# arihantb2/direct_lidar_odometry

Measured on AMD Instinct MI355X. Metric: gicp_iterations_per_sec, higher is better.
Workload: dtype f64

## Files before the change

direct_lidar_odometry_amd/csrc/ngicp_pass_group.inc:

```
#ifndef NG_ROBUST
#define NG_ROBUST false
#define NG_ROBUST_DEFAULTED
#endif
  for (int item = group * 4 + wave; item < a.n_batches; item = a.n_batches) {
    typedef const int __attribute__((address_space(4))) * ConstBatchPtr;
    ConstBatchPtr brec = (ConstBatchPtr)(unsigned long long)a.batches + 2 * (size_t)item;
    const int2 it = make_int2(brec[0], brec[1]);
    typedef const float __attribute__((address_space(4))) * ConstBoxPtr;
    const unsigned int far_word = (unsigned int)((ConstBatchPtr)(unsigned long long)a.batch_far)[item >> 2];
    const bool far_before = ((far_word >> (8 * (item & 3))) & 0xffu) != 0;
    ConstBoxPtr bbp = (ConstBoxPtr)(unsigned long long)a.batch_boxes + 6 * (size_t)item;
    const float bb_c0 = bbp[0], bb_c1 = bbp[1], bb_c2 = bbp[2], bb_h0 = bbp[3], bb_h1 = bbp[4], bb_h2 = bbp[5];
    const int qbase = it.x, qcount = it.y, batch = item;
    float mybest = 3.4028234664e38f;
    int mypos = -1;
    const int i = qbase + lane;
    const bool mine = lane < qcount;
    NG_STAMP(1);
    const bool have_prev = NG_HAVE_LIN != 0;
    float4 sp = make_float4(0.f, 0.f, 0.f, 0.f);
    int j_old = -1;
    float4 bp_old = make_float4(0.f, 0.f, 0.f, 0.f);
    double k4 = 0.0;
    double Mold[6] = {0, 0, 0, 0, 0, 0};
    if (mine) {
      sp = a.qpts[i];
      if (have_prev) {
        bp_old = tpt_old[i];
        j_old = __float_as_int(bp_old.w);
      }
      if (do_err) {
        const double* M = mahal_old + (size_t)i * 6;
#pragma unroll
        for (int e = 0; e < 6; ++e) Mold[e] = M[e];
      }
    }
    int Y0 = 0, Z0 = 0, wy = 1, grow = 0, nlive = 0;
    int b0x = 0, b0y = 0, b0z = 0, b1x = 0, b1y = 0, b1z = 0;
    bool list_rows = false;
    int rs[kStageRowsPerLane], rn[kStageRowsPerLane], rho[kStageRowsPerLane], ryz[kStageRowsPerLane], rk[kStageRowsPerLane];
    if (do_lin && !(a.mode & 8) && a.stage_grow >= 2 && (have_prev ? far_before : (a.mode & 32) != 0)) {
      {
        const float bcx = bb_c0, bcy = bb_c1, bcz = bb_c2, bhx = bb_h0, bhy = bb_h1, bhz = bb_h2;
        const float3 m = transform_point_rowmajor_f(Tf, bcx, bcy, bcz);
        const float mx = m.x, my = m.y, mz = m.z;
        const float pad = 1e-3f * g.h;
        const float ex = (fabsf(Tf[0]) * bhx + fabsf(Tf[1]) * bhy) + fabsf(Tf[2]) * bhz + pad + 4e-6f * (fabsf(mx) + bhx + bhy + bhz);
        const float ey = (fabsf(Tf[4]) * bhx + fabsf(Tf[5]) * bhy) + fabsf(Tf[6]) * bhz + pad + 4e-6f * (fabsf(my) + bhx + bhy + bhz);
        const float ez = (fabsf(Tf[8]) * bhx + fabsf(Tf[9]) * bhy) + fabsf(Tf[10]) * bhz + pad + 4e-6f * (fabsf(mz) + bhx + bhy + bhz);
        cell_coords(g, mx - ex, my - ey, mz - ez, b0x, b0y, b0z);
        cell_coords(g, mx + ex, my + ey, mz + ez, b1x, b1y, b1z);
      }
      int rows, X0 = 0, XS = 1;
      for (grow = a.stage_grow;; --grow) {
        X0 = max(b0x - grow, 0);
        Y0 = max(b0y - grow, 0);
        Z0 = max(b0z - grow, 0);
        const int X1 = min(b1x + grow, g.nx - 1), Y1 = min(b1y + grow, g.ny - 1), Z1 = min(b1z + grow, g.nz - 1);
        XS = X1 - X0 + 1;
        wy = Y1 - Y0 + 1;
        rows = wy * (Z1 - Z0 + 1);
        if ((rows <= kStageRows && XS <= kStageXs) || grow == 2) break;
      }
      if (rows <= kStageRows && XS <= kStageXs) {
        int sv[kStageRowsPerLane], ev[kStageRowsPerLane], ka[kStageRowsPerLane], kb[kStageRowsPerLane];
#pragma unroll
        for (int k = 0; k < kStageRowsPerLane; ++k) {
          const int r = lane + 64 * k;
          const bool has = r < rows;
          const int ry = Y0 + (has ? r : 0) % wy, rz = Z0 + (has ? r : 0) / wy;
          const int* rowp = a.tgt_cell_start + ((rz * g.ny + ry) * g.nx + X0);
          sv[k] = rowp[0];
          ev[k] = rowp[XS];
          ka[k] = rowp[b0x - X0];
          kb[k] = rowp[b1x + 1 - X0];
          rho[k] = max(max(b0y - ry, ry - b1y), max(max(b0z - rz, rz - b1z), 0));
          ryz[k] = ry | (rz << 16);
        }
        static_assert(kStageRowsPerLane == 4, "the four rows of a lane, spelled out for the compiler");
        asm volatile("" ::"v"(sv[0]), "v"(sv[1]), "v"(sv[2]), "v"(sv[3]), "v"(kb[0]), "v"(kb[1]), "v"(kb[2]), "v"(kb[3]));
#pragma unroll
        for (int k = 0; k < kStageRowsPerLane; ++k) {
          const bool has = lane + 64 * k < rows;
          rs[k] = sv[k];
          rn[k] = has ? ev[k] - sv[k] : 0;
          rk[k] = min(ka[k] - sv[k], 0xffff) | (min(kb[k] - sv[k], 0xffff) << 16);
        }
        list_rows = true;
      }
    }
    if (mine) {
      if (do_err && j_old >= 0) {
        const double ax = (double)sp.x, ay = (double)sp.y, az = (double)sp.z;
        const double tax = R[0] * ax + R[1] * ay + R[2] * az + t[0];
        const double tay = R[3] * ax + R[4] * ay + R[5] * az + t[1];
        const double taz = R[6] * ax + R[7] * ay + R[8] * az + t[2];
        const double ex = (double)bp_old.x - tax, ey = (double)bp_old.y - tay, ez = (double)bp_old.z - taz;
        if constexpr (NG_ROBUST) {
          k4 = err_term_robust(a.robust_kind, a.robust_c, a.robust_c2, ex, ey, ez, Mold);
        } else {
        const double m00 = Mold[0], m01 = Mold[1], m02 = Mold[2], m11 = Mold[3], m12 = Mold[4], m22 = Mold[5];
        const double mex = m00 * ex + m01 * ey + m02 * ez;
        const double mey = m01 * ex + m11 * ey + m12 * ez;
        const double mez = m02 * ex + m12 * ey + m22 * ez;
        k4 = ex * mex + ey * mey + ez * mez;
        }
      }
    }

    if (do_lin && (a.mode & 8)) {
      mypos = (qbase + lane) % 1000;
      mybest = 0.01f;
    } else if (do_lin) {
      const int qi = qbase + grp;
      const bool qok = grp < qcount;
      const float qpx = __shfl(sp.x, grp), qpy = __shfl(sp.y, grp), qpz = __shfl(sp.z, grp);
      const int jp = __shfl(j_old, grp);
      float4 bpo;
      bpo.x = __shfl(bp_old.x, grp); bpo.y = __shfl(bp_old.y, grp); bpo.z = __shfl(bp_old.z, grp); bpo.w = 0.f;
      float qx = 0.f, qy = 0.f, qz = 0.f;
      int cx = 0, cy = 0, cz = 0;
      if (qok) {
        const float3 q = transform_point_rowmajor_f(Tf, qpx, qpy, qpz);
        qx = q.x, qy = q.y, qz = q.z;
        cell_coords(g, qx, qy, qz, cx, cy, cz);
      }
      float best = 3.4028234664e38f;
      int pos = -1;
      if (qok && jp >= 0) {
        best = sqdist(qx, qy, qz, bpo);
        pos = jp;
      }
      NG_STAMP(2);
      bool listed = false;
      if (list_rows) {
        {
          wave_lds_sync();
          for (int lev = 0; lev <= grow; ++lev) {
#pragma unroll
            for (int k = 0; k < kStageRowsPerLane; ++k) {
              const bool on = rn[k] > 0 && rho[k] == lev;
              const unsigned long long m = __ballot(on);
              if (on) S.live[nlive + __popcll(m & ((1ull << lane) - 1ull))] = make_int4(ryz[k], rn[k], rs[k], rk[k]);
              nlive += __popcll(m);
            }
          }
          listed = true;
        }
      }
      NG_STAMP(3);
      if (a.dbg_stamps && lane == 0) {
        unsigned long long* d = a.dbg_stamps + (size_t)(blockIdx.x * 4 + wave) * kStampStride;
        d[10] = (unsigned long long)(listed ? grow : 0);
        d[11] = (unsigned long long)nlive;
        d[12] = (unsigned long long)qcount;
        d[13] = (unsigned long long)((b1x - b0x + 1) | ((b1y - b0y + 1) << 8) | ((b1z - b0z + 1) << 16));
      }
      bool went_far = false;
      const bool in_box = qok && listed && cx >= b0x && cx <= b1x && cy >= b0y && cy <= b1y && cz >= b0z && cz <= b1z;
      unsigned int dbg_g1 = 0, dbg_g2 = 0;
      auto pack_key = [](float d, int p) { return ((unsigned long long)__float_as_uint(d) << 32) | (unsigned int)p; };
      if (qok && sub == 0) {
        if (in_box) ++nstaged;
        S.qtab[grp] = make_float4(qx, qy, qz, 0.f);
        S.qkey[grp] = pack_key(best, pos);
      }
      if (lane == 0) S.q_tail = 0, S.q_head = 0;
      if (a.dbg_qstats && lane < 32) S.qstat[lane][0] = S.qstat[lane][1] = S.qstat[lane][2] = 0;
      wave_lds_sync();
      if (qok) {
        const float lim = fminf(best, a.gate_sq_f);
        constexpr int kRowsPerLane = (9 + G - 1) / G;
        struct alignas(4) Bounds4 { int v[4]; };
        Bounds4 bnd[kRowsPerLane], bxs[kRowsPerLane];
        float gap[kRowsPerLane];
        int code[kRowsPerLane];
#pragma unroll
        for (int k = 0; k < kRowsPerLane; ++k) {
          const int order = sub + k * G;
          const int tt = order == 0 ? 4 : (order < 5 ? 2 * order - 1 : (order == 5 ? 0 : (order == 6 ? 2 : (order == 7 ? 6 : 8))));
          const int z = cz + tt / 3 - 1, y = cy + tt % 3 - 1;
          code[k] = -1;
          gap[k] = 0.f;
          bnd[k] = Bounds4{{0, 0, 0, 0}};
          bxs[k] = Bounds4{{0, 0, 0, 0}};
          if (order < 9 && z >= 0 && z < g.nz && y >= 0 && y < g.ny) {
            gap[k] = row_gap_sq(g, y, z, cy, cz, qy, qz);
            if (gap[k] <= lim) {
              code[k] = tt;
              bnd[k] = *reinterpret_cast<const Bounds4*>(a.tgt_cell_start + ((z * g.ny + y) * g.nx + cx - 1));
              if (a.tgt_cell_box) bxs[k] = *reinterpret_cast<const Bounds4*>(a.tgt_cell_box + ((z * g.ny + y) * g.nx + cx - 1));
            }
          }
        }
        const float fx = fminf(fmaxf((qx - (g.ox + (float)cx * g.h)) * g.inv_h, 0.f), 1.f);
        int ntail = 0;
#pragma unroll
        for (int k = 0; k < kRowsPerLane; ++k) {
          const int s0 = cx > 0 ? bnd[k].v[0] : bnd[k].v[1], e0 = cx < g.nx - 1 ? bnd[k].v[3] : bnd[k].v[2];
          bool has = code[k] >= 0 && e0 > s0;
          if (has && a.tgt_cell_box) {
            unsigned int ub = (unsigned int)bxs[k].v[1];
            if (cx > 0) ub = cell_box_union(ub, (unsigned int)bxs[k].v[0]);
            if (cx < g.nx - 1) ub = cell_box_union(ub, (unsigned int)bxs[k].v[2]);
            gap[k] = fmaxf(gap[k], box_gap_sq(g, cy + code[k] % 3 - 1, cz + code[k] / 3 - 1, ub, qy, qz));
            has = gap[k] <= lim;
          }
          const unsigned long long hm = __ballot(has);
          if (has) {
            const int m = (jp >= s0 && jp < e0) ? jp : bnd[k].v[1] + (int)(fx * (float)(bnd[k].v[2] - bnd[k].v[1]));
            const int slot = ntail + __popcll(hm & ((1ull << lane) - 1ull));
            S.unit_q[slot] = grp | (code[k] << 5) | (min(max(m - s0, 0), (1 << 22) - 1) << 9);
            S.unit_s[slot] = s0;
            S.unit_e[slot] = e0;
            S.unit_g[slot] = gap[k];
          }
          ntail += __popcll(hm);
        }
        if (lane == 0) S.q_tail = ntail, S.q_head = 64 / kWalkLanes;
      }
      wave_lds_sync();
      int li_pre = sub;
      bool pre_far = false;
#if NGICP_PRE_FAR
      if (listed) {
        if (in_box) {
          const float b1 = unexplored_bound_sq(g, qx, qy, qz, cx, cy, cz, 1);
          pre_far = !(best <= b1 || b1 >= a.gate_sq_f);
        }
        if (__any(pre_far)) {
          if (pre_far) {
            const float lim = fminf(best, a.gate_sq_f);
            const float fxb = fminf(fmaxf((qx - (g.ox + (float)b0x * g.h)) / ((float)(b1x + 1 - b0x) * g.h), 0.f), 1.f);
            for (; li_pre < nlive; li_pre += G) {
              const int4 rec = S.live[li_pre];
              const float gp = row_gap_sq(g, rec.x & 0xffff, rec.x >> 16, cy, cz, qy, qz);
              if (gp > lim) continue;
              const int slot = atomicAdd(&S.q_tail, 1);
              if (slot >= kUnitCap) break;
              const int k0 = rec.w & 0xffff, k1 = (int)((unsigned int)rec.w >> 16);
              S.unit_q[slot] = grp | (9 << 5) | (min(max(k0 + (int)(fxb * (float)(k1 - k0)), 0), (1 << 22) - 1) << 9);
              S.unit_s[slot] = rec.z;
              S.unit_e[slot] = rec.z + rec.y;
              S.unit_g[slot] = gp;
            }
          }
          wave_lds_sync();
        }
      }
#endif
      NG_STAMP(16);
      {
        const int tail = min(S.q_tail, kUnitCap);
        unsigned int popped = 0;
        constexpr int kWalkers = 64 / kWalkLanes;
        const int ql = lane % kWalkLanes;
        auto next_unit = [&]() {
          if (tail <= kWalkers) return tail;
          if constexpr (kWalkLanes == 1) {
            return atomicAdd(&S.q_head, 1);
          } else {
            int nu = 0;
            if (ql == 0) nu = atomicAdd(&S.q_head, 1);
            return quad_perm_i<0x00>(nu);
          }
        };
        for (int u = lane / kWalkLanes; u < tail; u = next_unit()) {
          ++popped;
          const int uq = S.unit_q[u], qs = uq & 31, s0 = S.unit_s[u], e0 = S.unit_e[u];
          const float gyz = S.unit_g[u];
          const float4 q = S.qtab[qs];
          const unsigned long long k0 = S.qkey[qs];
          float ub = __uint_as_float((unsigned int)(k0 >> 32));
          int up = (int)(unsigned int)k0;
          if (gyz > fminf(ub, a.gate_sq_f)) continue;
          const unsigned int c_before = ncand;
          const unsigned int steps_before1 = dbg_g1;
          if constexpr (kWalkLanes == 1) scan_global_outward<kWin, kSideStep>(a.tgt3, s0, e0, s0 + (uq >> 9), q.x, q.y, q.z, gyz, a.gate_sq_f, ub, up, ncand, dbg_g1);
          else scan_quad_outward<kWin, kSideStep>(a.tgt3, s0, e0, s0 + (uq >> 9), q.x, q.y, q.z, gyz, a.gate_sq_f, ub, up, ncand, dbg_g1, ql);
          if (ql == 0) {
            if (a.dbg_qstats) atomicAdd(reinterpret_cast<int*>(a.dbg_qstats + a.n_src) + min((int)((dbg_g1 - steps_before1) & 0xffff), 63), 1);
            atomicMin(&S.qkey[qs], pack_key(ub, up));
            if (a.dbg_qstats) {
              atomicAdd(&S.qstat[qs][0], (int)(ncand - c_before));
              atomicAdd(&S.qstat[qs][1], 1);
            }
          }
        }
        NG_STAMP(17);
        if (a.dbg_stamps) {
          unsigned long long* d = a.dbg_stamps + (size_t)(blockIdx.x * 4 + wave) * kStampStride;
          atomicMax(&d[18], (unsigned long long)popped);
          if (lane == 0) d[19] = (unsigned long long)tail;
        }
      }
      wave_lds_sync();
      if (qok) {
        const unsigned long long k1 = S.qkey[grp];
        best = __uint_as_float((unsigned int)(k1 >> 32));
        pos = (int)(unsigned int)k1;
      }
      NG_STAMP(4);
      float bound1 = 0.f;
      if (qok) {
        bound1 = unexplored_bound_sq(g, qx, qy, qz, cx, cy, cz, 1);
        went_far = !(best <= bound1 || bound1 >= a.gate_sq_f);
      }
      const unsigned int dbg_c1 = ncand;
      unsigned int dbg_rows = 0;
      const bool need_far = in_box && went_far;
      if (listed && __any(need_far && (!pre_far || li_pre < nlive))) {
        int li = pre_far ? li_pre : sub;
        bool more = need_far;
        for (;;) {
          if (lane == 0) S.q_tail = 0, S.q_head = 0;
          wave_lds_sync();
          if (more) {
            const float lim = fminf(best, a.gate_sq_f);
            for (; li < nlive; li += G) {
              const int4 rec = S.live[li];
              if (row_gap_sq(g, rec.x & 0xffff, rec.x >> 16, cy, cz, qy, qz) > lim) continue;
              const int slot = atomicAdd(&S.q_tail, 1);
              if (slot >= kUnitCap) break;
              S.unit_q[slot] = grp | (li << 5);
              ++dbg_rows;
            }
            more = li < nlive;
          }
          wave_lds_sync();
          {
            const int tail = min(S.q_tail, kUnitCap);
            const int ql = lane % kWalkLanes;
            for (;;) {
              int u = 0;
              if (ql == 0) u = atomicAdd(&S.q_head, 1);
              if constexpr (kWalkLanes > 1) u = quad_perm_i<0x00>(u);
              if (u >= tail) break;
              const int unit = S.unit_q[u], qs = unit & 31;
              const int4 rec = S.live[unit >> 5];
              const float4 q = S.qtab[qs];
              int ux, uy, uz;
              cell_coords(g, q.x, q.y, q.z, ux, uy, uz);
              const float gyz = row_gap_sq(g, rec.x & 0xffff, rec.x >> 16, uy, uz, q.y, q.z);
              const unsigned long long k0 = S.qkey[qs];
              float ub = __uint_as_float((unsigned int)(k0 >> 32));
              int up = (int)(unsigned int)k0;
              if (gyz > fminf(ub, a.gate_sq_f)) continue;
              const int s0 = rec.z + (rec.w & 0xffff), e0 = rec.z + (int)((unsigned int)rec.w >> 16);
              const float frac3 = fminf(fmaxf((q.x - (g.ox + (float)b0x * g.h)) / ((float)(b1x + 1 - b0x) * g.h), 0.f), 1.f);
              const unsigned int c_before = ncand;
              const unsigned int steps_before2 = dbg_g2;
              if constexpr (kWalkLanes == 1) scan_global_outward<kWin, kSideStep>(a.tgt3, rec.z, rec.z + rec.y, s0 + (int)(frac3 * (float)(e0 - s0)), q.x, q.y, q.z, gyz, a.gate_sq_f, ub, up, ncand, dbg_g2);
              else scan_quad_outward<kWin, kSideStep>(a.tgt3, rec.z, rec.z + rec.y, s0 + (int)(frac3 * (float)(e0 - s0)), q.x, q.y, q.z, gyz, a.gate_sq_f, ub, up, ncand, dbg_g2, ql);
              if (ql == 0) {
                if (a.dbg_qstats) atomicAdd(reinterpret_cast<int*>(a.dbg_qstats + a.n_src) + 64 + min((int)((dbg_g2 - steps_before2) & 0xffff), 63), 1);
                atomicMin(&S.qkey[qs], pack_key(ub, up));
                if (a.dbg_qstats) {
                  atomicAdd(&S.qstat[qs][2], (int)(ncand - c_before));
                  atomicAdd(&S.qstat[qs][1], 1 << 16);
                }
              }
            }
          }
          wave_lds_sync();
          if (in_box) {
            const unsigned long long k1 = S.qkey[grp];
            best = __uint_as_float((unsigned int)(k1 >> 32));
            pos = (int)(unsigned int)k1;
          }
          if (!__any(more)) break;
        }
      }
      NG_STAMP(5);
      if (a.dbg_stamps && qok) {
        unsigned long long* d = a.dbg_stamps + (size_t)(blockIdx.x * 4 + wave) * kStampStride;
        atomicMax(&d[14], ((unsigned long long)(dbg_g2 & 0xffff) << 48) | ((unsigned long long)(dbg_g2 >> 16) << 32) | ((unsigned long long)dbg_rows << 16) | (ncand - dbg_c1));
        atomicMax(&d[15], ((unsigned long long)(dbg_g1 & 0xffff) << 48) | ((unsigned long long)(dbg_g1 >> 16) << 32) | dbg_c1);
      }
      const unsigned int c_before_shells = ncand;
      if (qok) nn_shells<G>(g, a.tgt3, a.tgt_cell_start, qx, qy, qz, cx, cy, cz, a.gate_sq_f, sub, need_far ? grow : 1, best, pos, ncand);
      if (a.dbg_qstats) {
        if (qok) atomicAdd(&S.qstat[grp][2], (int)(ncand - c_before_shells));
        wave_lds_sync();
        if (qok && sub == 0) a.dbg_qstats[qi] = make_int4(S.qstat[grp][0], S.qstat[grp][1], S.qstat[grp][2], (went_far ? 1 : 0) | (in_box ? 2 : 0) | (pos >= 0 ? 4 : 0));
      }
      {
        const bool any_far = __any(went_far);
        if (lane == 0) a.batch_far[batch] = any_far ? 1 : 0;
      }
      NG_STAMP(6);
      const int src_lane = (lane % B) * G;
      mybest = __shfl(best, src_lane);
      mypos = __shfl(pos, src_lane);
    }
    double acc[kNumSums];
#pragma unroll
    for (int v = 0; v < kNumSums; ++v) acc[v] = 0.0;
    if ((a.mode & 16) && mine) {
      tpt_new[i] = make_float4(0.f, 0.f, 0.f, __int_as_float(mypos));
      acc[27] += (double)mybest;
    } else if (mine) {
      const double ax = (double)sp.x, ay = (double)sp.y, az = (double)sp.z;
      const double tax = R[0] * ax + R[1] * ay + R[2] * az + t[0];
      const double tay = R[3] * ax + R[4] * ay + R[5] * az + t[1];
      const double taz = R[6] * ax + R[7] * ay + R[8] * az + t[2];

      acc[28] += k4;
      if (do_lin) {
        const int pos = mypos;
        const bool valid = (pos >= 0) && ((double)mybest < a.gate_sq);
        if (!valid) tpt_new[i] = make_float4(0.f, 0.f, 0.f, __int_as_float(-1));
        if (valid) {
          ++nvalid;
          const double* CB = a.cov_tgt + (size_t)pos * 6;
          const double* CA = a.cov_src + (size_t)__float_as_int(sp.w) * 6;
          const Xyz bp = a.tgt3[pos];
          double ca[6];
#pragma unroll
          for (int e = 0; e < 6; ++e) ca[e] = CA[e];
          tpt_new[i] = make_float4(bp.x, bp.y, bp.z, __int_as_float(pos));
          double rcr[6], M[6];
          rotate_sym(R, ca, rcr);
#pragma unroll
          for (int e = 0; e < 6; ++e) rcr[e] = CB[e] + rcr[e];
          inv3_sym(rcr, M);
          double* Mo = mahal_new + (size_t)i * 6;
#pragma unroll
          for (int e = 0; e < 6; ++e) Mo[e] = M[e];

          const double ex = (double)bp.x - tax, ey = (double)bp.y - tay, ez = (double)bp.z - taz;
          if constexpr (NG_ROBUST) lin_terms_robust(acc, a.robust_kind, a.robust_c, a.robust_c2, tax, tay, taz, ex, ey, ez, M);
          else lin_terms(acc, tax, tay, taz, ex, ey, ez, M);
        }
      }
    }
    {
      double* red = S.red;
      double out = 0.0;
#pragma unroll
      for (int half = 0; half < 2; ++half) {
        wave_lds_sync();
        if ((lane >> 4) == half) {
#pragma unroll
          for (int v = 0; v < kNumSums; ++v) red[(lane & 15) * 30 + v] = acc[v];
        }
        wave_lds_sync();
        if (lane < kNumSums)
          for (int l = 0; l < 16; ++l) out += red[l * 30 + lane];
      }
      if (lane < kNumSums) wave_total += out;
    }
  }

  NG_STAMP(7);
  {
    wave_lds_sync();
    unsigned int* cnt = reinterpret_cast<unsigned int*>(S.red);
    cnt[lane] = ncand;
    cnt[64 + lane] = nvalid;
    cnt[128 + lane] = nstaged;
    wave_lds_sync();
    if (lane >= kNumSums && lane < kNumSlots) {
      unsigned int sum = 0;
      for (int l = 0; l < 64; ++l) sum += cnt[(lane - kNumSums) * 64 + l];
      wave_total = (double)sum;
    }
    if (lane < kNumSlots) lds[wave][lane] = wave_total;
  }
  NG_STAMP(8);
  __syncthreads();
  NG_STAMP(9);
  if (threadIdx.x < kNumSlots) {
    const int v = threadIdx.x;
    const double val = ((lds[0][v] + lds[1][v]) + lds[2][v]) + lds[3][v];
    if (FUSED) __hip_atomic_store(a.partials + (size_t)group * kNumSlots + v, val, __ATOMIC_RELAXED, __HIP_MEMORY_SCOPE_AGENT);
    else a.partials[(size_t)group * kNumSlots + v] = val;
  }
  if (a.dbg_span && threadIdx.x == 0) {
    unsigned long long* d = a.dbg_span + (size_t)blockIdx.x * 4;
    d[1] = __builtin_amdgcn_s_memrealtime();
    d[2] = (unsigned long long)__builtin_amdgcn_s_getreg((31 << 11) | 4) | ((unsigned long long)__builtin_amdgcn_s_getreg((31 << 11) | 20) << 32);
    d[3] = (unsigned long long)(unsigned int)group;
  }
  if (a.grp_cost && threadIdx.x == 0) {
    const int cost = (int)min((__builtin_amdgcn_s_memtime() - t_start) >> 4, 0x7fffffffull);
    if (FUSED) __hip_atomic_store(a.grp_cost + group, cost, __ATOMIC_RELAXED, __HIP_MEMORY_SCOPE_AGENT);
    else a.grp_cost[group] = cost;
  }
#ifdef NG_ROBUST_DEFAULTED
#undef NG_ROBUST
#undef NG_ROBUST_DEFAULTED
#endif
```

direct_lidar_odometry_amd/csrc/ngicp_search.h:

```cpp
#pragma once
#include "ngicp_grid.h"

namespace ngk {

struct alignas(4) Xyz { float x, y, z; };
__device__ __forceinline__ float sqdist(float qx, float qy, float qz, const Xyz& p) {
  const float dx = qx - p.x, dy = qy - p.y, dz = qz - p.z;
  float r = dx * dx;
  r = r + dy * dy;
  r = r + dz * dz;
  return r;
}

__device__ __forceinline__ float3 transform_point_rowmajor_f(const float* Tf, float x, float y, float z) {
  float3 q;
  q.x = ((Tf[0] * x + Tf[1] * y) + Tf[2] * z) + Tf[3];
  q.y = ((Tf[4] * x + Tf[5] * y) + Tf[6] * z) + Tf[7];
  q.z = ((Tf[8] * x + Tf[9] * y) + Tf[10] * z) + Tf[11];
  return q;
}

__global__ void __launch_bounds__(256) k_pack_pos(const float4* __restrict__ in, int n_padded, int pad, float4* __restrict__ out) {
  const int i = blockIdx.x * blockDim.x + threadIdx.x;
  if (i >= n_padded) return;
  const float4 p = in[i];
  const bool real = i >= pad && i < n_padded - pad;
  out[i] = make_float4(p.x, p.y, p.z, __int_as_float(real ? i - pad : -1));
}

__global__ void __launch_bounds__(256) k_pack_xyz(const float4* __restrict__ in, int n, Xyz* __restrict__ out) {
  const int i = blockIdx.x * blockDim.x + threadIdx.x;
  if (i >= n) return;
  const float4 p = in[i];
  out[i] = Xyz{p.x, p.y, p.z};
}

template <int G>
__device__ __forceinline__ void group_min(float& d, int& p) {
#pragma unroll
  for (int o = G / 2; o > 0; o >>= 1) {
    const float od = __shfl_xor(d, o);
    const int op = __shfl_xor(p, o);
    const bool take = (od < d) || (od == d && (unsigned)op < (unsigned)p);
    d = take ? od : d;
    p = take ? op : p;
  }
}

__device__ __forceinline__ bool nn_better(float d, int p, float best, int bestp) { return d < best || (d == best && (unsigned)p < (unsigned)bestp); }

constexpr int kStageRowsPerLane = 4;
constexpr int kStageRows = 64 * kStageRowsPerLane;
constexpr int kStageXs = 20;
constexpr int kStageMaxGrow = 6;

#ifndef NGICP_PASS_WAVES
#define NGICP_PASS_WAVES 3
#endif
#ifndef NGICP_WALK_WINDOW
#define NGICP_WALK_WINDOW 12
#endif

#ifndef NGICP_WALK_PREFETCH
#define NGICP_WALK_PREFETCH 0
#endif
#ifndef NGICP_PRE_FAR
#define NGICP_PRE_FAR 0
#endif
#ifndef NGICP_ALIGNED_WINDOWS
#define NGICP_ALIGNED_WINDOWS 0
#endif
constexpr int kWalkWindow = NGICP_WALK_WINDOW;
static_assert(kWalkWindow <= kSortedPad && kWalkWindow % 2 == 0, "walk windows may overhang the array by at most the sentinel frame");

constexpr int kUnitCap = 288;

struct WaveStage {
  union {
    struct {
      int4 live[kStageRows];
      int qstat[32][3];
    };
    double red[16 * 30];
  };
  unsigned long long qkey[32];
  float4 qtab[32];
  int unit_q[kUnitCap], unit_s[kUnitCap], unit_e[kUnitCap];
  float unit_g[kUnitCap];
  int q_tail, q_head;
};

__device__ __forceinline__ void wave_lds_sync() {
  __builtin_amdgcn_fence(__ATOMIC_RELEASE, "wavefront");
  __builtin_amdgcn_wave_barrier();
  __builtin_amdgcn_fence(__ATOMIC_ACQUIRE, "wavefront");
}

template <int W = kWalkWindow, int kStep = kWalkWindow, class PT>
__device__ __forceinline__ void scan_global_outward(const PT* __restrict__ tgt, int s, int e, int m, float qx, float qy, float qz, float gyz, float gate_sq,
                                                    float& best, int& pos, unsigned int& ncand, unsigned int& gsteps) {
  if (e <= s) return;
  gsteps += 0x10000u;
  m = min(max(m, s), e - 1);
  constexpr bool kQuadLoads = NGICP_ALIGNED_WINDOWS && sizeof(PT) == 12 && W % 4 == 0 && kStep % 4 == 0;
  const int w0 = kQuadLoads ? ((m - W / 2) & ~3) : m - W / 2;
  int w = w0, dir = 0, lo = w0, hi = w0 + W;
  int wn = W;
  static_assert(kStep >= 2 && kStep <= W, "side windows are at most as long as the first");
  bool go_left = false;
  for (;;) {
    const PT* __restrict__ q = tgt + w;
    PT c[W];
    if constexpr (kQuadLoads) {
      const float4* __restrict__ q4 = reinterpret_cast<const float4*>(q);
      float4 r[3 * W / 4];
#pragma unroll
      for (int j = 0; j < 3 * W / 4; ++j)
        if (j < 3 * kStep / 4 || wn == W) r[j] = q4[j];
#pragma unroll
      for (int j = 0; j < W / 4; ++j) {
        if (j < kStep / 4 || wn == W) {
          const float4 r0 = r[3 * j], r1 = r[3 * j + 1], r2 = r[3 * j + 2];
          c[4 * j].x = r0.x; c[4 * j].y = r0.y; c[4 * j].z = r0.z;
          c[4 * j + 1].x = r0.w; c[4 * j + 1].y = r1.x; c[4 * j + 1].z = r1.y;
          c[4 * j + 2].x = r1.z; c[4 * j + 2].y = r1.w; c[4 * j + 2].z = r2.x;
          c[4 * j + 3].x = r2.y; c[4 * j + 3].y = r2.z; c[4 * j + 3].z = r2.w;
        }
      }
    } else {
#pragma unroll
      for (int j = 0; j < W; ++j)
        if (j < kStep || wn == W) c[j] = q[j];
    }
    unsigned int pf = 0;
    if constexpr (NGICP_WALK_PREFETCH != 0) {
      if (dir >= 0 && hi < e) pf ^= *reinterpret_cast<const unsigned int*>(tgt + (hi + (NGICP_WALK_PREFETCH > 1 ? kStep - 1 : 0)));
      if (dir <= 0 && lo > s) pf ^= *reinterpret_cast<const unsigned int*>(tgt + (lo - (NGICP_WALK_PREFETCH > 1 ? kStep : 1)));
    }
    float lb = sqdist(qx, qy, qz, c[0]);
    int lj = 0;
#pragma unroll
    for (int j = 1; j < W; ++j) {
      if (j < kStep || wn == W) {
        const float d = sqdist(qx, qy, qz, c[j]);
        if (d < lb) { lb = d; lj = j; }
      }
    }
    if (nn_better(lb, w + lj, best, pos)) { best = lb; pos = w + lj; }
    ncand += wn;
    ++gsteps;
    if constexpr (NGICP_WALK_PREFETCH != 0) gsteps += (pf == 0x7fc0beefu) ? 0x100u : 0u;
    const float lim = fminf(best, gate_sq), dr = (wn == W ? c[W - 1].x : c[kStep - 1].x) - qx, dl = qx - c[0].x;
    const bool more_right = hi < e && !(dr > 0.f && dr * dr + gyz > lim);
    const bool more_left = lo > s && !(dl > 0.f && dl * dl + gyz > lim);
    if (dir == 0) go_left = more_left;
    if (dir >= 0 && more_right) {
      dir = 1;
      w = hi;
      hi += kStep;
      wn = kStep;
    } else if (dir >= 0 ? go_left : more_left) {
      dir = -1;
      lo -= kStep;
      w = lo;
      wn = kStep;
    } else {
      break;
    }
  }
}

#ifndef NGICP_WALK_LANES
#define NGICP_WALK_LANES 1
#endif
constexpr int kWalkLanes = NGICP_WALK_LANES;
template <int CTRL>
__device__ __forceinline__ int quad_perm_i(int v) { return __builtin_amdgcn_update_dpp(v, v, CTRL, 0xf, 0xf, false); }
template <int CTRL>
__device__ __forceinline__ float quad_perm_f(float v) { return __int_as_float(quad_perm_i<CTRL>(__float_as_int(v))); }
template <int W, int kStep, class PT>
__device__ __forceinline__ void scan_quad_outward(const PT* __restrict__ tgt, int s, int e, int m, float qx, float qy, float qz, float gyz, float gate_sq,
                                                  float& best, int& pos, unsigned int& ncand, unsigned int& gsteps, int ql) {
  static_assert(W % 4 == 0 && kStep % 4 == 0 && kStep >= 4 && kStep <= W, "windows are dealt to the four lanes of a quad");
  constexpr int PER = W / 4, PERS = kStep / 4;
  if (e <= s) return;
  gsteps += 0x10000u;
  m = min(max(m, s), e - 1);
  int w = m - W / 2, dir = 0, lo = m - W / 2, hi = m - W / 2 + W;
  int wn = W;
  bool go_left = false;
  for (;;) {
    const PT* __restrict__ q = tgt + (w + ql);
    PT c[PER];
#pragma unroll
    for (int j = 0; j < PER; ++j)
      if (j < PERS || wn == W) c[j] = q[4 * j];
    float lb = sqdist(qx, qy, qz, c[0]);
    int lj = 0;
#pragma unroll
    for (int j = 1; j < PER; ++j) {
      if (j < PERS || wn == W) {
        const float d = sqdist(qx, qy, qz, c[j]);
        if (d < lb) { lb = d; lj = j; }
      }
    }
    int lp = w + ql + 4 * lj;
    const float xl = quad_perm_f<0x00>(c[0].x), xr = quad_perm_f<0xff>(wn == W ? c[PER - 1].x : c[PERS - 1].x);
    {
      const float od = quad_perm_f<0xb1>(lb);
      const int op = quad_perm_i<0xb1>(lp);
      if (nn_better(od, op, lb, lp)) { lb = od; lp = op; }
    }
    {
      const float od = quad_perm_f<0x4e>(lb);
      const int op = quad_perm_i<0x4e>(lp);
      if (nn_better(od, op, lb, lp)) { lb = od; lp = op; }
    }
    if (nn_better(lb, lp, best, pos)) { best = lb; pos = lp; }
    if (ql == 0) ncand += wn;
    ++gsteps;
    const float lim = fminf(best, gate_sq), dr = xr - qx, dl = qx - xl;
    const bool more_right = hi < e && !(dr > 0.f && dr * dr + gyz > lim);
    const bool more_left = lo > s && !(dl > 0.f && dl * dl + gyz > lim);
    if (dir == 0) go_left = more_left;
    if (dir >= 0 && more_right) {
      dir = 1;
      w = hi;
      hi += kStep;
      wn = kStep;
    } else if (dir >= 0 ? go_left : more_left) {
      dir = -1;
      lo -= kStep;
      w = lo;
      wn = kStep;
    } else {
      break;
    }
  }
}

template <int G, class PT>
__device__ __forceinline__ void nn_shells(const Grid& g, const PT* __restrict__ tgt, const int* __restrict__ cell_start, float qx, float qy, float qz,
                                          int cx, int cy, int cz, float gate_sq_f, int sub, int rdone, float& best, int& pos, unsigned int& ncand) {
  const int rmax = max(max(g.nx, g.ny), g.nz);
  unsigned int steps = 0;
  for (int r = rdone;; ++r) {
    const float bound = unexplored_bound_sq(g, qx, qy, qz, cx, cy, cz, r);
    if (best <= bound || bound >= gate_sq_f || r >= rmax) break;
    const int R = r + 1;
    const int z0 = max(cz - R, 0), z1 = min(cz + R, g.nz - 1);
    const int y0 = max(cy - R, 0), y1 = min(cy + R, g.ny - 1);
    const int xa = max(cx - R, 0), xb = min(cx + R, g.nx - 1);
    const bool lo = cx - R >= 0, hi = cx + R <= g.nx - 1;
    const int wy = y1 - y0 + 1;
    const int nrows = wy * (z1 - z0 + 1);
    const float xfrac = fminf(fmaxf((qx - (g.ox + (float)xa * g.h)) / ((float)(xb + 1 - xa) * g.h), 0.f), 1.f);
    for (int t0 = sub; t0 < nrows; t0 += 4 * G) {
      int s0[4], e0[4], s1[4], e1[4];
      float gap[4];
      const float lim = fminf(best, gate_sq_f);
#pragma unroll
      for (int u = 0; u < 4; ++u) {
        const int t = t0 + u * G;
        const bool ok = t < nrows;
        const int z = z0 + (ok ? t : 0) / wy, y = y0 + (ok ? t : 0) % wy;
        const int row = (z * g.ny + y) * g.nx;
        const bool face = z == cz - R || z == cz + R || y == cy - R || y == cy + R;
        gap[u] = row_gap_sq(g, y, z, cy, cz, qy, qz);
        const bool want = ok && gap[u] <= lim;
        const int a0 = face ? xa : cx - R, a1 = face ? xb + 1 : cx - R + 1;
        const bool use0 = want && (face || lo), use1 = want && !face && hi;
        s0[u] = use0 ? cell_start[row + a0] : 0;
        e0[u] = use0 ? cell_start[row + a1] : 0;
        s1[u] = use1 ? cell_start[row + cx + R] : (face ? -1 : 0);
        e1[u] = use1 ? cell_start[row + cx + R + 1] : 0;
      }
#pragma unroll 1
      for (int u = 0; u < 4; ++u) {
        int a0 = s0[0], b0 = e0[0], a1 = s1[0], b1 = e1[0];
        float gp = gap[0];
#pragma unroll
        for (int v = 1; v < 4; ++v)
          if (u == v) a0 = s0[v], b0 = e0[v], a1 = s1[v], b1 = e1[v], gp = gap[v];
        if (gp > fminf(best, gate_sq_f)) continue;
        if (b0 > a0) scan_global_outward(tgt, a0, b0, a1 < 0 ? a0 + (int)(xfrac * (float)(b0 - a0)) : b0 - 1, qx, qy, qz, gp, gate_sq_f, best, pos, ncand, steps);
        if (b1 > a1 && a1 >= 0) scan_global_outward(tgt, a1, b1, a1, qx, qy, qz, gp, gate_sq_f, best, pos, ncand, steps);
      }
    }
    if (G > 1) group_min<G>(best, pos);
  }
}

}
```

Before: 21040.

## Unify far-row queueing with ballot compaction and share the unit drain loop

Far-row units are now enqueued with a ballot/popcount prefix instead of a per-lane LDS atomicAdd, and two rows are processed per step. Far rows now carry the same precomputed start, end, mid and gap as the pre-far units, so a single shared drain loop replaces the separate far-walk loop and its per-unit row recomputation. The intent is to remove LDS atomic contention and duplicated work in the far search phase. Optional timing stamps and an LDS size static_assert are added; unit ordering and overflow handling change, which could alter load balance.

```diff
diff --git a/direct_lidar_odometry_amd/csrc/ngicp_pass_group.inc b/direct_lidar_odometry_amd/csrc/ngicp_pass_group.inc
--- a/direct_lidar_odometry_amd/csrc/ngicp_pass_group.inc
+++ b/direct_lidar_odometry_amd/csrc/ngicp_pass_group.inc
@@ -1,6 +1,33 @@
 #ifndef NG_ROBUST
 #define NG_ROBUST false
 #define NG_ROBUST_DEFAULTED
+#endif
+#ifdef NGICP_FAR_STAMPS
+#define NG_FAR_STAMP_BEGIN() far_t0 = __builtin_amdgcn_s_memtime()
+#define NG_FAR_STAMP_QUEUED(n)                                  \
+  do {                                                          \
+    const unsigned long long now = __builtin_amdgcn_s_memtime(); \
+    far_enq += now - far_t0, far_t0 = now;                      \
+    far_units += (unsigned long long)(n), ++far_rounds;         \
+  } while (0)
+#define NG_FAR_STAMP_DRAINED()                                  \
+  do {                                                          \
+    const unsigned long long now = __builtin_amdgcn_s_memtime(); \
+    far_drn += now - far_t0, far_t0 = now;                      \
+  } while (0)
+#define NG_FAR_STAMP_END()                                                                               \
+  do {                                                                                                   \
+    if (a.dbg_stamps && lane == 0) {                                                                     \
+      unsigned long long* d = a.dbg_stamps + (size_t)(blockIdx.x * 4 + wave) * kStampStride;             \
+      d[20] = far_enq | (far_units << 40);                                                               \
+      d[21] = far_drn | (far_rounds << 48);                                                              \
+    }                                                                                                    \
+  } while (0)
+#else
+#define NG_FAR_STAMP_BEGIN() do {} while (0)
+#define NG_FAR_STAMP_QUEUED(n) do {} while (0)
+#define NG_FAR_STAMP_DRAINED() do {} while (0)
+#define NG_FAR_STAMP_END() do {} while (0)
 #endif
   for (int item = group * 4 + wave; item < a.n_batches; item = a.n_batches) {
     typedef const int __attribute__((address_space(4))) * ConstBatchPtr;
@@ -220,40 +247,47 @@
         if (lane == 0) S.q_tail = ntail, S.q_head = 64 / kWalkLanes;
       }
       wave_lds_sync();
-      int li_pre = sub;
-      bool pre_far = false;
-#if NGICP_PRE_FAR
-      if (listed) {
-        if (in_box) {
-          const float b1 = unexplored_bound_sq(g, qx, qy, qz, cx, cy, cz, 1);
-          pre_far = !(best <= b1 || b1 >= a.gate_sq_f);
-        }
-        if (__any(pre_far)) {
-          if (pre_far) {
-            const float lim = fminf(best, a.gate_sq_f);
-            const float fxb = fminf(fmaxf((qx - (g.ox + (float)b0x * g.h)) / ((float)(b1x + 1 - b0x) * g.h), 0.f), 1.f);
-            for (; li_pre < nlive; li_pre += G) {
-              const int4 rec = S.live[li_pre];
-              const float gp = row_gap_sq(g, rec.x & 0xffff, rec.x >> 16, cy, cz, qy, qz);
-              if (gp > lim) continue;
-              const int slot = atomicAdd(&S.q_tail, 1);
-              if (slot >= kUnitCap) break;
-              const int k0 = rec.w & 0xffff, k1 = (int)((unsigned int)rec.w >> 16);
+      unsigned int dbg_rows = 0;
+      auto queue_listed_rows = [&](const int base, const bool active, int& li_io, const float lim) -> int {
+        constexpr int kRowsPerStep = 2;
+        const float fxb = fminf(fmaxf((qx - (g.ox + (float)b0x * g.h)) / ((float)(b1x + 1 - b0x) * g.h), 0.f), 1.f);
+        const unsigned long long below = (1ull << lane) - 1ull;
+        int ntail = base;
+        while (ntail < kUnitCap) {
+          int4 rec[kRowsPerStep];
+          bool on[kRowsPerStep];
+#pragma unroll
+          for (int k = 0; k < kRowsPerStep; ++k) {
+            const int idx = li_io + k * G;
+            on[k] = active && idx < nlive;
+            rec[k] = S.live[on[k] ? idx : 0];
+          }
+          if (!__any(on[0])) break;
+          bool taken = true;
+#pragma unroll
+          for (int k = 0; k < kRowsPerStep; ++k) {
+            const float gp = row_gap_sq(g, rec[k].x & 0xffff, rec[k].x >> 16, cy, cz, qy, qz);
+            const bool want = on[k] && taken && gp <= lim;
+            const unsigned long long m = __ballot(want);
+            const int slot = ntail + __popcll(m & below);
+            if (want && slot < kUnitCap) {
+              const int k0 = rec[k].w & 0xffff, k1 = (int)((unsigned int)rec[k].w >> 16);
               S.unit_q[slot] = grp | (9 << 5) | (min(max(k0 + (int)(fxb * (float)(k1 - k0)), 0), (1 << 22) - 1) << 9);
-              S.unit_s[slot] = rec.z;
-              S.unit_e[slot] = rec.z + rec.y;
+              S.unit_s[slot] = rec[k].z;
+              S.unit_e[slot] = rec[k].z + rec[k].y;
               S.unit_g[slot] = gp;
+              ++dbg_rows;
             }
-          }
-          wave_lds_sync();
-        }
-      }
-#endif
-      NG_STAMP(16);
-      {
-        const int tail = min(S.q_tail, kUnitCap);
+            taken = taken && on[k] && !(want && slot >= kUnitCap);
+            if (taken) li_io += G;
+            ntail += __popcll(m);
+          }
+        }
+        return min(ntail, kUnitCap);
+      };
+      constexpr int kWalkers = 64 / kWalkLanes;
+      auto drain_units = [&](const int tail, unsigned int& steps, const int hist_at, const int stat_at, const int stat_one) -> unsigned int {
         unsigned int popped = 0;
-        constexpr int kWalkers = 64 / kWalkLanes;
         const int ql = lane % kWalkLanes;
         auto next_unit = [&]() {
           if (tail <= kWalkers) return tail;
@@ -275,18 +309,40 @@
           int up = (int)(unsigned int)k0;
           if (gyz > fminf(ub, a.gate_sq_f)) continue;
           const unsigned int c_before = ncand;
-          const unsigned int steps_before1 = dbg_g1;
-          if constexpr (kWalkLanes == 1) scan_global_outward<kWin, kSideStep>(a.tgt3, s0, e0, s0 + (uq >> 9), q.x, q.y, q.z, gyz, a.gate_sq_f, ub, up, ncand, dbg_g1);
-          else scan_quad_outward<kWin, kSideStep>(a.tgt3, s0, e0, s0 + (uq >> 9), q.x, q.y, q.z, gyz, a.gate_sq_f, ub, up, ncand, dbg_g1, ql);
+          const unsigned int steps_before = steps;
+          if constexpr (kWalkLanes == 1) scan_global_outward<kWin, kSideStep>(a.tgt3, s0, e0, s0 + (uq >> 9), q.x, q.y, q.z, gyz, a.gate_sq_f, ub, up, ncand, steps);
+          else scan_quad_outward<kWin, kSideStep>(a.tgt3, s0, e0, s0 + (uq >> 9), q.x, q.y, q.z, gyz, a.gate_sq_f, ub, up, ncand, steps, ql);
           if (ql == 0) {
-            if (a.dbg_qstats) atomicAdd(reinterpret_cast<int*>(a.dbg_qstats + a.n_src) + min((int)((dbg_g1 - steps_before1) & 0xffff), 63), 1);
+            if (a.dbg_qstats) atomicAdd(reinterpret_cast<int*>(a.dbg_qstats + a.n_src) + hist_at + min((int)((steps - steps_before) & 0xffff), 63), 1);
             atomicMin(&S.qkey[qs], pack_key(ub, up));
             if (a.dbg_qstats) {
-              atomicAdd(&S.qstat[qs][0], (int)(ncand - c_before));
-              atomicAdd(&S.qstat[qs][1], 1);
+              atomicAdd(&S.qstat[qs][stat_at], (int)(ncand - c_before));
+              atomicAdd(&S.qstat[qs][1], stat_one);
             }
           }
         }
+        return popped;
+      };
+      int li_pre = sub;
+      bool pre_far = false;
+#if NGICP_PRE_FAR
+      if (listed) {
+        if (in_box) {
+          const float b1 = unexplored_bound_sq(g, qx, qy, qz, cx, cy, cz, 1);
+          pre_far = !(best <= b1 || b1 >= a.gate_sq_f);
+        }
+        if (__any(pre_far)) {
+          const int ntail = queue_listed_rows(min(S.q_tail, kUnitCap), pre_far, li_pre, fminf(best, a.gate_sq_f));
+          wave_lds_sync();
+          if (lane == 0) S.q_tail = ntail;
+          wave_lds_sync();
+        }
+      }
+#endif
+      NG_STAMP(16);
+      {
+        const int tail = min(S.q_tail, kUnitCap);
+        const unsigned int popped = drain_units(tail, dbg_g1, 0, 0, 1);
         NG_STAMP(17);
         if (a.dbg_stamps) {
           unsigned long long* d = a.dbg_stamps + (size_t)(blockIdx.x * 4 + wave) * kStampStride;
@@ -307,71 +363,33 @@
         went_far = !(best <= bound1 || bound1 >= a.gate_sq_f);
       }
       const unsigned int dbg_c1 = ncand;
-      unsigned int dbg_rows = 0;
+#ifdef NGICP_FAR_STAMPS
+      unsigned long long far_t0 = 0, far_enq = 0, far_drn = 0, far_units = 0, far_rounds = 0;
+#endif
       const bool need_far = in_box && went_far;
       if (listed && __any(need_far && (!pre_far || li_pre < nlive))) {
         int li = pre_far ? li_pre : sub;
         bool more = need_far;
+        NG_FAR_STAMP_BEGIN();
         for (;;) {
-          if (lane == 0) S.q_tail = 0, S.q_head = 0;
+          const int tail = queue_listed_rows(0, more, li, fminf(best, a.gate_sq_f));
+          more = more && li < nlive;
+          if (lane == 0) S.q_head = kWalkers;
           wave_lds_sync();
-          if (more) {
-            const float lim = fminf(best, a.gate_sq_f);
-            for (; li < nlive; li += G) {
-              const int4 rec = S.live[li];
-              if (row_gap_sq(g, rec.x & 0xffff, rec.x >> 16, cy, cz, qy, qz) > lim) continue;
-              const int slot = atomicAdd(&S.q_tail, 1);
-              if (slot >= kUnitCap) break;
-              S.unit_q[slot] = grp | (li << 5);
-              ++dbg_rows;
-            }
-            more = li < nlive;
-          }
-          wave_lds_sync();
-          {
-            const int tail = min(S.q_tail, kUnitCap);
-            const int ql = lane % kWalkLanes;
-            for (;;) {
-              int u = 0;
-              if (ql == 0) u = atomicAdd(&S.q_head, 1);
-              if constexpr (kWalkLanes > 1) u = quad_perm_i<0x00>(u);
-              if (u >= tail) break;
-              const int unit = S.unit_q[u], qs = unit & 31;
-              const int4 rec = S.live[unit >> 5];
-              const float4 q = S.qtab[qs];
-              int ux, uy, uz;
-              cell_coords(g, q.x, q.y, q.z, ux, uy, uz);
-              const float gyz = row_gap_sq(g, rec.x & 0xffff, rec.x >> 16, uy, uz, q.y, q.z);
-              const unsigned long long k0 = S.qkey[qs];
-              float ub = __uint_as_float((unsigned int)(k0 >> 32));
-              int up = (int)(unsigned int)k0;
-              if (gyz > fminf(ub, a.gate_sq_f)) continue;
-              const int s0 = rec.z + (rec.w & 0xffff), e0 = rec.z + (int)((unsigned int)rec.w >> 16);
-              const float frac3 = fminf(fmaxf((q.x - (g.ox + (float)b0x * g.h)) / ((float)(b1x + 1 - b0x) * g.h), 0.f), 1.f);
-              const unsigned int c_before = ncand;
-              const unsigned int steps_before2 = dbg_g2;
-              if constexpr (kWalkLanes == 1) scan_global_outward<kWin, kSideStep>(a.tgt3, rec.z, rec.z + rec.y, s0 + (int)(frac3 * (float)(e0 - s0)), q.x, q.y, q.z, gyz, a.gate_sq_f, ub, up, ncand, dbg_g2);
-              else scan_quad_outward<kWin, kSideStep>(a.tgt3, rec.z, rec.z + rec.y, s0 + (int)(frac3 * (float)(e0 - s0)), q.x, q.y, q.z, gyz, a.gate_sq_f, ub, up, ncand, dbg_g2, ql);
-              if (ql == 0) {
-                if (a.dbg_qstats) atomicAdd(reinterpret_cast<int*>(a.dbg_qstats + a.n_src) + 64 + min((int)((dbg_g2 - steps_before2) & 0xffff), 63), 1);
-                atomicMin(&S.qkey[qs], pack_key(ub, up));
-                if (a.dbg_qstats) {
-                  atomicAdd(&S.qstat[qs][2], (int)(ncand - c_before));
-                  atomicAdd(&S.qstat[qs][1], 1 << 16);
-                }
-              }
-            }
-          }
+          NG_FAR_STAMP_QUEUED(tail);
+          drain_units(tail, dbg_g2, 64, 2, 1 << 16);
           wave_lds_sync();
           if (in_box) {
             const unsigned long long k1 = S.qkey[grp];
             best = __uint_as_float((unsigned int)(k1 >> 32));
             pos = (int)(unsigned int)k1;
           }
+          NG_FAR_STAMP_DRAINED();
           if (!__any(more)) break;
         }
       }
       NG_STAMP(5);
+      NG_FAR_STAMP_END();
       if (a.dbg_stamps && qok) {
         unsigned long long* d = a.dbg_stamps + (size_t)(blockIdx.x * 4 + wave) * kStampStride;
         atomicMax(&d[14], ((unsigned long long)(dbg_g2 & 0xffff) << 48) | ((unsigned long long)(dbg_g2 >> 16) << 32) | ((unsigned long long)dbg_rows << 16) | (ncand - dbg_c1));
@@ -487,6 +505,10 @@
     if (FUSED) __hip_atomic_store(a.grp_cost + group, cost, __ATOMIC_RELAXED, __HIP_MEMORY_SCOPE_AGENT);
     else a.grp_cost[group] = cost;
   }
+#undef NG_FAR_STAMP_BEGIN
+#undef NG_FAR_STAMP_QUEUED
+#undef NG_FAR_STAMP_DRAINED
+#undef NG_FAR_STAMP_END
 #ifdef NG_ROBUST_DEFAULTED
 #undef NG_ROBUST
 #undef NG_ROBUST_DEFAULTED
diff --git a/direct_lidar_odometry_amd/csrc/ngicp_search.h b/direct_lidar_odometry_amd/csrc/ngicp_search.h
--- a/direct_lidar_odometry_amd/csrc/ngicp_search.h
+++ b/direct_lidar_odometry_amd/csrc/ngicp_search.h
@@ -89,6 +89,8 @@
   float unit_g[kUnitCap];
   int q_tail, q_head;
 };
+static_assert(sizeof(WaveStage) <= 9872 && 4 * sizeof(WaveStage) + 4 * 32 * sizeof(double) <= 40 * 1024 + 512,
+              "four of these and the block's row of sums are the pass kernel's 40 KB of LDS per block: more, and a CU holds a block less");
 
 __device__ __forceinline__ void wave_lds_sync() {
   __builtin_amdgcn_fence(__ATOMIC_RELEASE, "wavefront");
```

Measured after the change: 21940, median of 6. 4.3% higher.
